# MatteoMer/zolt

Measured on AMD Instinct MI355X. Metric: BN254 G1 MSM/sec, higher is better.
Workload: dtype u32; 1 GPU; msm_g1_2^20; points=1048576, points_per_gpu=1048576, streams=3, window_bits=17, windows=15, table_levels=15, table_bytes=1006632960, mode=precomputed table of multiples

## Files before the change

### zolt_amd/csrc/g1_29.hip.h

```cpp
#pragma once
#include "fp29.hip.h"
#include "g1.hip.h"

namespace zg {

struct XYZZ29 {
    F29 x, y, zz, zzz;
};

ZG_DEV XYZZ xyzz29_to_std(const XYZZ29 &a, bool inf) {
    if (inf) return XYZZ::identity();
    XYZZ r;
    r.x = f29_to_fp(a.x); r.y = f29_to_fp(a.y); r.zz = f29_to_fp(a.zz); r.zzz = f29_to_fp(a.zzz);
    return r;
}
ZG_DEV void xyzz29_from_std(const XYZZ &s, XYZZ29 &a, bool &inf) {
    inf = s.is_identity();
    a.x = f29_from_fp(s.x); a.y = f29_from_fp(s.y); a.zz = f29_from_fp(s.zz); a.zzz = f29_from_fp(s.zzz);
}

ZG_DEV void xyzz29_start(XYZZ29 &a, const F29 &px, const F29 &py) {
    a.x = px; a.y = py;
#pragma unroll
    for (int i = 0; i < 9; i++) { a.zz.l[i] = Fp29::ONE[i]; a.zzz.l[i] = Fp29::ONE[i]; }
}

ZG_DEV u32 xyzz29_madd_nz(XYZZ29 &a, const F29 &px, const F29 &py, u32 neg) {
#ifdef ZG_F29_SERIAL
    F29 U2 = f29_mul(px, a.zz);
    F29 S2 = f29_mul(py, a.zzz);
#else
    F29 U2, S2;
    f29_mul_x2(U2, px, a.zz, S2, py, a.zzz);
#endif
    F29 Pp = f29_sub7(U2, a.x);
    F29 R = f29_pmsub45(S2, a.y, neg);
    u32 exc = 0;
#ifndef ZG_EXP_NOSLOW
    if (f29_is_zero_modp(Pp)) exc = f29_is_zero_modp(R) ? 2u : 1u;
#endif
#ifdef ZG_F29_SERIAL
    F29 PP = f29_sqr(Pp);
    F29 PPP = f29_mul(Pp, PP);
    F29 Q = f29_mul(a.x, PP);
    F29 X3 = f29_x3(f29_sqr(R), PPP, Q);
    F29 Y3 = f29_mul2(R, f29_sub7(Q, X3), f29_neg4(a.y), PPP);
    a.zz = f29_mul(a.zz, PP);
    a.zzz = f29_mul(a.zzz, PPP);
    a.x = X3;
    a.y = Y3;
#else
    F29 PP, RR, PPP, Q, ZZ3, Y3, ZZZ3;
    f29_sqr_x2(PP, Pp, RR, R);
    f29_mul_x3(PPP, Pp, PP, Q, a.x, PP, ZZ3, a.zz, PP);
    F29 X3 = f29_x3(RR, PPP, Q);
    f29_mul2_mul(Y3, R, f29_sub7(Q, X3), f29_neg4(a.y), PPP, ZZZ3, a.zzz, PPP);
    a.x = X3;
    a.y = Y3;
    a.zz = ZZ3;
    a.zzz = ZZZ3;
#endif
    return exc;
}
ZG_DEV void xyzz29_madd_except(XYZZ29 &a, bool &inf, const F29 &px, const F29 &py, u32 neg, u32 exc) {
    if (exc == 2u) {
        Affine q;
        q.x = f29_to_fp(px); q.y = f29_to_fp(neg ? f29_neg2(py) : py);
        xyzz29_from_std(xyzz_dbl_affine(q), a, inf);
    } else {
        inf = true;
    }
}

ZG_DEV void xyzz29_madd(XYZZ29 &a, bool &inf, const F29 &px, const F29 &py) {
    if (inf) {
        xyzz29_start(a, px, py);
        inf = false;
        return;
    }
    u32 exc = xyzz29_madd_nz(a, px, py, 0u);
    if (exc) xyzz29_madd_except(a, inf, px, py, 0u, exc);
}

ZG_DEV XYZZ29 xyzz29_identity() {
    XYZZ29 r;
#pragma unroll
    for (int i = 0; i < 9; i++) { r.x.l[i] = 0; r.y.l[i] = 0; r.zz.l[i] = 0; r.zzz.l[i] = 0; }
    return r;
}
ZG_DEV bool xyzz29_is_identity(const XYZZ29 &a) { return f29_all_zero(a.zz); }

ZG_DEV XYZZ29 xyzz29_from_std_val(const XYZZ &s) {
    if (s.is_identity()) return xyzz29_identity();
    XYZZ29 a;
    a.x = f29_from_fp(s.x); a.y = f29_from_fp(s.y); a.zz = f29_from_fp(s.zz); a.zzz = f29_from_fp(s.zzz);
    return a;
}
ZG_DEV XYZZ xyzz29_to_std_val(const XYZZ29 &a) { return xyzz29_to_std(a, xyzz29_is_identity(a)); }

ZG_DEV XYZZ29 xyzz29_dbl(const XYZZ29 &p) {
    if (xyzz29_is_identity(p)) return p;
    F29 U = f29_times2(p.y);
    F29 V = f29_sqr(U);
    F29 W = f29_mul(U, V);
    F29 S = f29_mul(p.x, V);
    F29 M = f29_times3(f29_sqr(p.x));
    XYZZ29 r;
    r.x = f29_sub4_2c(f29_sqr(M), S);
    r.y = f29_mul2(M, f29_sub7(S, r.x), W, f29_neg4(p.y));
    r.zz = f29_mul(V, p.zz);
    r.zzz = f29_mul(W, p.zzz);
    return r;
}

struct Jac29 {
    F29 x, y, z;
};
ZG_DEV Jac29 jac29_dbl(const Jac29 &p) {
    F29 A = f29_sqr(p.x);
    F29 B = f29_sqr(p.y);
    F29 B4 = f29_times4(B);
    F29 D = f29_mul(p.x, B4);
    F29 E = f29_times3(A);
    F29 F = f29_sqr(E);
    Jac29 r;
    r.x = f29_sub4_2c(F, D);
    r.y = f29_mul2(E, f29_sub7(D, r.x), f29_neg2(B), f29_times2(B4));
    r.z = f29_mul(f29_times2(p.y), p.z);
    return r;
}

ZG_DEV XYZZ29 xyzz29_add(const XYZZ29 &a, const XYZZ29 &b) {
    if (xyzz29_is_identity(a)) return b;
    if (xyzz29_is_identity(b)) return a;
    F29 U1 = f29_mul(a.x, b.zz);
    F29 U2 = f29_mul(b.x, a.zz);
    F29 S1 = f29_mul(a.y, b.zzz);
    F29 S2 = f29_mul(b.y, a.zzz);
    F29 Pp = f29_sub2(U2, U1);
    F29 R = f29_sub2(S2, S1);
    if (f29_is_zero_modp(Pp)) {
        if (f29_is_zero_modp(R)) return xyzz29_dbl(a);
        return xyzz29_identity();
    }
    F29 PP = f29_sqr(Pp);
    F29 PPP = f29_mul(Pp, PP);
    F29 Q = f29_mul(U1, PP);
    XYZZ29 r;
    r.x = f29_x3(f29_sqr(R), PPP, Q);
    r.y = f29_mul2(R, f29_sub7(Q, r.x), f29_neg2(S1), PPP);
    r.zz = f29_mul(f29_mul(a.zz, b.zz), PP);
    r.zzz = f29_mul(f29_mul(a.zzz, b.zzz), PPP);
    return r;
}

ZG_DEV XYZZ29 xyzz29_load(const void *p) {
    const uint4 *q = reinterpret_cast<const uint4 *>(p);
    u32 w[36];
#pragma unroll
    for (int i = 0; i < 9; i++) {
        uint4 v = q[i];
        w[4 * i] = v.x; w[4 * i + 1] = v.y; w[4 * i + 2] = v.z; w[4 * i + 3] = v.w;
    }
    XYZZ29 r;
#pragma unroll
    for (int i = 0; i < 9; i++) { r.x.l[i] = w[i]; r.y.l[i] = w[9 + i]; r.zz.l[i] = w[18 + i]; r.zzz.l[i] = w[27 + i]; }
    return r;
}
ZG_DEV void xyzz29_store(void *p, const XYZZ29 &v) {
    u32 w[36];
#pragma unroll
    for (int i = 0; i < 9; i++) { w[i] = v.x.l[i]; w[9 + i] = v.y.l[i]; w[18 + i] = v.zz.l[i]; w[27 + i] = v.zzz.l[i]; }
    uint4 *q = reinterpret_cast<uint4 *>(p);
#pragma unroll
    for (int i = 0; i < 9; i++) q[i] = make_uint4(w[4 * i], w[4 * i + 1], w[4 * i + 2], w[4 * i + 3]);
}
ZG_DEV XYZZ29 xyzz29_shfl_down(const XYZZ29 &v, int delta) {
    XYZZ29 r;
#pragma unroll
    for (int i = 0; i < 9; i++) {
        r.x.l[i] = __shfl_down(v.x.l[i], delta, 64);
        r.y.l[i] = __shfl_down(v.y.l[i], delta, 64);
        r.zz.l[i] = __shfl_down(v.zz.l[i], delta, 64);
        r.zzz.l[i] = __shfl_down(v.zzz.l[i], delta, 64);
    }
    return r;
}

}
```

### zolt_amd/csrc/msm.hip

```cpp
#include <string.h>

#include <mutex>
#include <vector>

#include "common.hip.h"
#include "g1.hip.h"
#include "g1_29.hip.h"
#include "g1_29x4.hip.h"
#include "msm_plan.h"

#ifndef ZG_TAIL_PRIO
#define ZG_TAIL_PRIO 3
#endif
#define ZG_HIPRIO() __builtin_amdgcn_s_setprio(ZG_TAIL_PRIO)

struct zg_bases_s {
    size_t n = 0;
    int device = -1;
    zg::MsmPlan plan;
    char *d_table = nullptr;
    uint8_t *d_inf = nullptr;
    uint64_t *d_scal = nullptr;
    struct Lane {
        uint32_t *d_dig = nullptr, *d_sorted = nullptr, *d_hist = nullptr, *d_starts = nullptr;
// ... 672 lines not shown
#else
#define ZG_ROW_MASK 0x7FFFFFFFu
#endif
#ifdef ZG_EXP_ACC_WAVES
#define ZG_ACC_ATTR __attribute__((amdgpu_waves_per_eu(ZG_EXP_ACC_WAVES, ZG_EXP_ACC_WAVES)))
#else
#define ZG_ACC_ATTR __attribute__((amdgpu_waves_per_eu(2, 2)))
#endif
struct Row29 {
    uint4 w[4];
};
ZG_DEV Row29 row29_load(const char *p) {
    Row29 r;
    const uint4 *q = reinterpret_cast<const uint4 *>(p);
#pragma unroll
    for (int i = 0; i < 4; i++) r.w[i] = q[i];
    return r;
}
ZG_DEV void row29_unpack(const Row29 &r, F29 &px, F29 &py) {
    const u32 x[8] = {r.w[0].x, r.w[0].y, r.w[0].z, r.w[0].w, r.w[1].x, r.w[1].y, r.w[1].z, r.w[1].w};
    const u32 y[8] = {r.w[2].x, r.w[2].y, r.w[2].z, r.w[2].w, r.w[3].x, r.w[3].y, r.w[3].z, r.w[3].w};
    px = f29_unpack(x);
    py = f29_unpack(y);
#pragma unroll
    for (int i = 0; i < 9; i++) {
        asm volatile("" : "+v"(px.l[i]));
        asm volatile("" : "+v"(py.l[i]));
    }
}

template <bool QUAD>
__global__ void __launch_bounds__(256) ZG_ACC_ATTR msm_accumulate_chunk_kernel(const uint32_t *sorted, const uint32_t *starts, const uint32_t *nzrank,
                                                                   const uint32_t *nzend, const char *table, uint32_t NK, uint32_t NT,
                                                                   char *part) {
    uint32_t i = blockIdx.x * blockDim.x + threadIdx.x, q = 0;
    if (QUAD) {
        q = i & 3;
        i >>= 2;
    }
    uint32_t total = starts[NK];
    uint32_t C = chunk_len(total, NT);
    uint64_t a64 = (uint64_t)i * C;
    if (i >= NT || a64 >= total) return;
    uint32_t a = (uint32_t)a64, b = a + C < total ? a + C : total;
    uint32_t lo = 0, hi = NK;
    while (hi - lo > 1) {
        uint32_t mid = (lo + hi) >> 1;
        if (starts[mid] <= a) lo = mid; else hi = mid;
    }
    uint32_t r = nzrank[lo], kend = starts[lo + 1];
#ifndef ZG_ACC_RUNEND_STARTS
    uint32_t knext = nzend[r + 1];
#endif
    XYZZ29 acc;
    bool acc_inf = true;
    uint32_t e = sorted[a];
    Row29 row = row29_load(table + 64 * (size_t)(e & ZG_ROW_MASK));
    uint32_t rneg = e >> 31;
    uint32_t e1 = a + 1 < b ? sorted[a + 1] : 0u;
    for (uint32_t p = a; p < b; p++) {
        F29 px, py;
#ifdef ZG_ACC_ROW_COPY
        Row29 nxt = row;
        uint32_t nneg = 0;
        if (p + 1 < b) {
            uint32_t e2 = e1;
            if (p + 2 < b) e1 = sorted[p + 2];
            nxt = row29_load(table + 64 * (size_t)(e2 & ZG_ROW_MASK));
            nneg = e2 >> 31;
        }
        row29_unpack(row, px, py);
        const uint32_t neg = 0u - rneg;
#else
        row29_unpack(row, px, py);
        const uint32_t neg = 0u - rneg;
        if (p + 1 < b) {
            uint32_t e2 = e1;
            if (p + 2 < b) e1 = sorted[p + 2];
            row = row29_load(table + 64 * (size_t)(e2 & ZG_ROW_MASK));
            rneg = e2 >> 31;
        }
#endif
        if (__builtin_expect(p == kend, 0)) {
            if (q == 0) xyzz29_store(part + 144 * (size_t)(i + r), acc_inf ? xyzz29_identity() : acc);
            acc_inf = true;
            r++;
#ifdef ZG_ACC_RUNEND_STARTS
            kend = starts[nzend[r] + 1];
#else
            asm volatile("v_mov_b32 %0, %1" : "=v"(kend) : "v"(knext));
            knext = nzend[r + 1];
#endif
        }
        uint32_t exc = 0;
        if (QUAD) {
            if (neg) py = f29_neg2(py);
            xyzz29_madd4(acc, acc_inf, px, py, q);
        } else if (__builtin_expect(acc_inf, 0)) {
            xyzz29_start(acc, px, neg ? f29_neg2(py) : py);
            acc_inf = false;
        } else {
#ifdef ZG_ACC_SIGN_BRANCH
            if (neg) py = f29_neg2(py);
            exc = xyzz29_madd_nz(acc, px, py, 0u);
        }
        if (__builtin_expect(exc != 0, 0)) xyzz29_madd_except(acc, acc_inf, px, py, 0u, exc);
#else
            exc = xyzz29_madd_nz(acc, px, py, neg);
        }
        if (__builtin_expect(exc != 0, 0)) xyzz29_madd_except(acc, acc_inf, px, py, neg, exc);
#endif
#ifdef ZG_ACC_ROW_COPY
        row = nxt;
        rneg = nneg;
#endif
    }
    if (q == 0) xyzz29_store(part + 144 * (size_t)(i + r), acc_inf ? xyzz29_identity() : acc);
}

__global__ void __launch_bounds__(64) msm_bucket_combine_kernel(const char *part, const uint32_t *starts, const uint32_t *nzrank, uint32_t NK,
                                                                uint32_t NT, int GS, char *buckets, uint32_t *heavy_list, MsmState *st) {
    ZG_HIPRIO();
    uint32_t t = (blockIdx.x * 64 + threadIdx.x) >> 2, q = threadIdx.x & 3;
    uint32_t k = t / (uint32_t)GS, g = t % (uint32_t)GS;
    XYZZ29 acc = xyzz29_identity();
    bool light = false;
    if (k < NK) {
        uint32_t C = chunk_len(starts[NK], NT);
        uint32_t s0 = starts[k], s1 = starts[k + 1];
        if (s1 == s0) {
            light = true;
        } else {
            uint32_t q0 = s0 / C, q1 = (s1 - 1) / C, cnt = q1 - q0 + 1, base = q0 + nzrank[k];
            if (cnt > 8u * (uint32_t)GS) {
                if (g == 0 && q == 0) {
                    if (cnt > HUGE_PARTIALS) heavy_list[NK + atomicAdd(&st->nhuge, 1u)] = k;
                    else heavy_list[atomicAdd(&st->nheavy, 1u)] = k;
                }
            } else {
                light = true;
                if (g < cnt) acc = xyzz29_load(part + 144 * (size_t)(base + g));
                uint32_t j = g + (uint32_t)GS;
                XYZZ29 nxt = j < cnt ? xyzz29_load(part + 144 * (size_t)(base + j)) : xyzz29_identity();
                while (j < cnt) {
                    XYZZ29 cur = nxt;
                    j += (uint32_t)GS;
                    if (j < cnt) nxt = xyzz29_load(part + 144 * (size_t)(base + j));
                    acc = xyzz29_add4(acc, cur, q);
                }
            }
        }
    }
    for (int d = 1; d < GS; d <<= 1) {
        XYZZ29 o = xyzz29_shfl_down(acc, 4 * d);
        if ((g & (uint32_t)(2 * d - 1)) == 0) acc = xyzz29_add4(acc, o, q);
    }
    if (light && g == 0 && q == 0) xyzz29_store(buckets + 144 * (size_t)k, acc);
}

__device__ __forceinline__ XYZZ29 block_sum_xyzz29(const XYZZ29 &acc, uint4 *sh) {
    uint32_t tid = threadIdx.x;
    xyzz29_store(&sh[tid * 9], acc);
    __syncthreads();
    if (tid < 128) {
        XYZZ29 x = xyzz29_load(&sh[tid * 9]), y = xyzz29_load(&sh[(tid + 128) * 9]);
        xyzz29_store(&sh[tid * 9], xyzz29_add(x, y));
    }
    __syncthreads();
    uint32_t g = tid >> 2, q = tid & 3;
    for (uint32_t o = 64; o > 0; o >>= 1) {
        if (g < o) {
            XYZZ29 x = xyzz29_load(&sh[g * 9]), y = xyzz29_load(&sh[(g + o) * 9]);
            XYZZ29 r = xyzz29_add4(x, y, q);
            if (q == 0) xyzz29_store(&sh[g * 9], r);
        }
        __syncthreads();
    }
    return xyzz29_load(&sh[0]);
}

__device__ __forceinline__ XYZZ29 wave_sum_xyzz29(const XYZZ29 &acc, uint4 *sh) {
    const uint32_t tid = threadIdx.x;
    xyzz29_store(&sh[tid * 9], acc);
    __syncthreads();
    if (tid < 32) {
        XYZZ29 x = xyzz29_load(&sh[tid * 9]), y = xyzz29_load(&sh[(tid + 32) * 9]);
        xyzz29_store(&sh[tid * 9], xyzz29_add(x, y));
    }
    __syncthreads();
    const uint32_t g = tid >> 2, q = tid & 3;
    for (uint32_t o = 16; o > 0; o >>= 1) {
        if (g < o) {
            XYZZ29 x = xyzz29_load(&sh[g * 9]), y = xyzz29_load(&sh[(g + o) * 9]);
            XYZZ29 r = xyzz29_add4(x, y, q);
            if (q == 0) xyzz29_store(&sh[g * 9], r);
        }
        __syncthreads();
    }
    return xyzz29_load(&sh[0]);
}

__global__ void __launch_bounds__(256) msm_heavy_kernel(const char *part, const uint32_t *starts, const uint32_t *nzrank, const uint32_t *nzlist,
                                                        uint32_t NK, uint32_t NT, const uint32_t *heavy_list, MsmState *st, char *part2,
                                                        char *buckets) {
    ZG_HIPRIO();
    __shared__ uint4 sh[256 * 9];
    __shared__ uint32_t sh_last;
    const uint32_t nheavy = st->nheavy, nhuge = st->nhuge;
    if (nheavy == 0 && nhuge == 0) return;
    const uint32_t C = chunk_len(starts[NK], NT), tid = threadIdx.x;
    {
        const uint32_t lane = tid & 63;
        for (uint32_t h = blockIdx.x * 4 + (tid >> 6); h < nheavy; h += gridDim.x * 4) {
            uint32_t k = heavy_list[h];
            uint32_t s0 = starts[k], s1 = starts[k + 1];
            uint32_t q0 = s0 / C, q1 = (s1 - 1) / C, cnt = q1 - q0 + 1, base = q0 + nzrank[k];
            XYZZ29 acc = xyzz29_identity();
            for (uint32_t j = lane; j < cnt; j += 64) acc = xyzz29_add(acc, xyzz29_load(part + 144 * (size_t)(base + j)));
            for (int d = 1; d < 64; d <<= 1) {
                XYZZ29 o = xyzz29_shfl_down(acc, d);
                if ((lane & (uint32_t)(2 * d - 1)) == 0) acc = xyzz29_add(acc, o);
            }
            if (lane == 0) xyzz29_store(buckets + 144 * (size_t)k, acc);
        }
    }
    if (nhuge == 0) return;
    const uint32_t *huge_list = heavy_list + NK;
    uint32_t *arrive = reinterpret_cast<uint32_t *>(st) + 4;
    uint32_t NZ = nzrank[NK];
    uint32_t lo_slot = blockIdx.x * HEAVY_BLOCK_ITEMS, hi_slot = lo_slot + HEAVY_BLOCK_ITEMS;
    if (lo_slot >= NT + NK) return;
    uint32_t lo = 0, hi = NZ;
    while (hi - lo > 1) {
        uint32_t mid = (lo + hi) >> 1;
        if (starts[nzlist[mid]] / C + mid <= lo_slot) lo = mid; else hi = mid;
    }
    for (uint32_t r = lo; r < NZ; r++) {
        uint32_t k = nzlist[r];
        uint32_t s0 = starts[k], s1 = starts[k + 1];
        uint32_t q0 = s0 / C, q1 = (s1 - 1) / C, cnt = q1 - q0 + 1, base = q0 + r;
        if (base >= hi_slot) break;
        if (cnt <= HUGE_PARTIALS || base + cnt <= lo_slot) continue;
        uint32_t r0 = base > lo_slot ? base : lo_slot, r1 = base + cnt < hi_slot ? base + cnt : hi_slot;
        XYZZ29 acc = xyzz29_identity();
        for (uint32_t j = r0 + tid; j < r1; j += 256) acc = xyzz29_add(acc, xyzz29_load(part + 144 * (size_t)j));
        XYZZ29 res = block_sum_xyzz29(acc, sh);
        const uint32_t b0 = base / HEAVY_BLOCK_ITEMS, b1 = (base + cnt - 1) / HEAVY_BLOCK_ITEMS;
        if (tid == 0) {
            xyzz29_store(part2 + 144 * (size_t)(blockIdx.x + r), res);
            uint32_t h = 0;
            while (h < nhuge && huge_list[h] != k) h++;
            uint32_t arrived = __hip_atomic_fetch_add(&arrive[h], 1u, __ATOMIC_ACQ_REL, __HIP_MEMORY_SCOPE_AGENT);
            asm volatile("s_waitcnt vmcnt(0)" ::: "memory");
            sh_last = arrived == b1 - b0 ? 1u : 0u;
        }
        __syncthreads();
        if (sh_last) {
            XYZZ29 a2 = xyzz29_identity();
            for (uint32_t bb = b0 + tid; bb <= b1; bb += 256) a2 = xyzz29_add(a2, xyzz29_load(part2 + 144 * (size_t)(bb + r)));
            __syncthreads();
            XYZZ29 tot = block_sum_xyzz29(a2, sh);
            if (tid == 0) xyzz29_store(buckets + 144 * (size_t)k, tot);
        }
        __syncthreads();
    }
}

__global__ void __launch_bounds__(256) msm_bitsum_kernel(const char *buckets, uint32_t NB, int c, char *out) {
    ZG_HIPRIO();
    __shared__ uint4 sh[256 * 9];
    uint32_t b = blockIdx.y, g = blockIdx.z, PB = gridDim.x;
    uint32_t total = (b == (uint32_t)(c - 1)) ? 1u : NB / 2;
    XYZZ29 acc = xyzz29_identity();
    for (uint32_t j = blockIdx.x * 256 + threadIdx.x; j < total; j += PB * 256) {
        uint32_t k = (b == (uint32_t)(c - 1)) ? NB : ((((j >> b) << 1) | 1u) << b) | (j & ((1u << b) - 1u));
        acc = xyzz29_add(acc, xyzz29_load(buckets + 144 * ((size_t)g * NB + (k - 1))));
    }
    XYZZ29 r = block_sum_xyzz29(acc, sh);
    if (threadIdx.x == 0) xyzz29_store(out + 144 * (((size_t)g * c + b) * PB + blockIdx.x), r);
}

__global__ void __launch_bounds__(256) msm_rowcol_kernel(const char *buckets, uint32_t NB, int lb, int hb, char *rc) {
    ZG_HIPRIO();
    __shared__ uint4 sh[256 * 9];
    const uint32_t x = blockIdx.x, g = blockIdx.y, nrow = 1u << hb, ncol = 1u << lb, t = threadIdx.x;
    XYZZ29 acc = xyzz29_identity();
    const uint32_t len = x < nrow ? ncol : nrow;
    for (uint32_t e = t; e < len; e += 256) {
        const uint32_t k = x < nrow ? ((x << lb) | e) : ((e << lb) | (x - nrow));
        if (k != 0) {
            XYZZ29 v = xyzz29_load(buckets + 144 * ((size_t)g * NB + (k - 1)));
            acc = e < 256 ? v : xyzz29_add(acc, v);
        }
    }
    XYZZ29 r = block_sum_xyzz29(acc, sh);
    if (t == 0) xyzz29_store(rc + 144 * ((size_t)g * (nrow + ncol) + x), r);
}
__global__ void __launch_bounds__(64) msm_rowcol_wave_kernel(const char *buckets, uint32_t NB, int lb, int hb, char *rc) {
    ZG_HIPRIO();
    __shared__ uint4 sh[64 * 9];
    const uint32_t x = blockIdx.x, g = blockIdx.y, nrow = 1u << hb, ncol = 1u << lb, t = threadIdx.x;
    XYZZ29 acc = xyzz29_identity();
    const uint32_t len = x < nrow ? ncol : nrow;
    bool first = true;
    for (uint32_t e = t; e < len; e += 64) {
        const uint32_t k = x < nrow ? ((x << lb) | e) : ((e << lb) | (x - nrow));
        if (k != 0) {
            XYZZ29 v = xyzz29_load(buckets + 144 * ((size_t)g * NB + (k - 1)));
            acc = first ? v : xyzz29_add(acc, v);
            first = false;
        }
    }
    XYZZ29 r = wave_sum_xyzz29(acc, sh);
    if (t == 0) xyzz29_store(rc + 144 * ((size_t)g * (nrow + ncol) + x), r);
}
static void launch_rowcol(hipStream_t st, const char *buckets, uint32_t NB, int lb, int hb, int sets, char *rc) {
    const int wave_from = env_int("ZG_MSM_ROWCOL_WAVE_FROM", 3);
    if (wave_from > 0 && sets >= wave_from)
        hipLaunchKernelGGL(msm_rowcol_wave_kernel, dim3((1u << hb) + (1u << lb), sets), dim3(64), 0, st, buckets, NB, lb, hb, rc);
    else
        hipLaunchKernelGGL(msm_rowcol_kernel, dim3((1u << hb) + (1u << lb), sets), dim3(256), 0, st, buckets, NB, lb, hb, rc);
}

__global__ void __launch_bounds__(256) msm_bits2d_kernel(const char *buckets, const char *rc, uint32_t NB, int c, int lb, int hb, char *out) {
    ZG_HIPRIO();
    __shared__ uint4 sh[256 * 9];
    const uint32_t b = blockIdx.x, g = blockIdx.y, nrow = 1u << hb, ncol = 1u << lb, t = threadIdx.x;
    const char *rcg = rc + 144 * (size_t)g * (nrow + ncol);
    XYZZ29 acc = xyzz29_identity();
    if (b == (uint32_t)(c - 1)) {
        if (t == 0) acc = xyzz29_load(buckets + 144 * ((size_t)g * NB + (NB - 1)));
    } else if (b < (uint32_t)lb) {
        for (uint32_t e = t; e < ncol; e += 256)
            if ((e >> b) & 1u) acc = xyzz29_add(acc, xyzz29_load(rcg + 144 * (size_t)(nrow + e)));
    } else {
        for (uint32_t e = t; e < nrow; e += 256)
            if ((e >> (b - (uint32_t)lb)) & 1u) acc = xyzz29_add(acc, xyzz29_load(rcg + 144 * (size_t)e));
    }
    XYZZ29 r = block_sum_xyzz29(acc, sh);
    if (t == 0) xyzz29_store(out + 144 * ((size_t)g * c + b), r);
}

ZG_DEV void write_result(const XYZZ &acc, int mode, uint64_t *out_rec, uint8_t *out_inf) {
    Affine r;
    bool inf = xyzz_to_affine(acc, r);
    if (mode == 0) {
        affine_store(out_rec, r);
        *out_inf = inf ? 1 : 0;
    } else {
        Fp one = Fp::one();
        if (inf) {
            fe_store(out_rec, one); fe_store(out_rec + 4, one); fe_store(out_rec + 8, Fp::zero());
        } else {
            fe_store(out_rec, r.x); fe_store(out_rec + 4, r.y); fe_store(out_rec + 8, one);
        }
    }
}

ZG_DEV void write_partial_unnormalised(const XYZZ &acc, uint64_t *out_rec) {
    Fp X, Y, Z;
    xyzz_to_jacobian(acc, X, Y, Z);
    fe_store(out_rec, X); fe_store(out_rec + 4, Y); fe_store(out_rec + 8, Z);
}

__global__ void __launch_bounds__(512) msm_final_kernel(const char *bits, int c, int PB, int G, char *rg, int mode, uint64_t *out_rec,
                                                        uint8_t *out_inf, uint32_t rec_stride, uint32_t inf_stride) {
    ZG_HIPRIO();
    __shared__ uint4 pts[256 * 9];
    uint32_t tid = threadIdx.x, g = blockIdx.x, quad = tid >> 2, q = tid & 3;
    uint32_t S = 1;
    while (S < (uint32_t)PB) S <<= 1;
    if (tid < 256) {
        uint32_t b = tid / S, j = tid % S;
        XYZZ29 v = xyzz29_identity();
        if (b < (uint32_t)c && j < (uint32_t)PB) v = xyzz29_load(bits + 144 * (((size_t)g * c + b) * PB + j));
        xyzz29_store(&pts[tid * 9], v);
    }
    __syncthreads();
    for (uint32_t d = 1; d < S; d <<= 1) {
        uint32_t per_bit = S / (2 * d);
        if (quad < (256 / S) * per_bit) {
            uint32_t b = quad / per_bit, j = (quad % per_bit) * 2 * d;
            XYZZ29 x = xyzz29_load(&pts[(b * S + j) * 9]), y = xyzz29_load(&pts[(b * S + j + d) * 9]);
            XYZZ29 r = xyzz29_add4(x, y, q);
            if (q == 0) xyzz29_store(&pts[(b * S + j) * 9], r);
        }
        __syncthreads();
    }
    if (quad < (uint32_t)c) {
        XYZZ29 v = xyzz29_load(&pts[(quad * S) * 9]);
#if !(defined(ZG_EXP_SKIP) && (ZG_EXP_SKIP & 1))
        for (uint32_t i = 0; i < quad; i++) v = xyzz29_dbl4(v, q);
// ... 626 lines not shown
            uint32_t *d_fbase = ln.d_fine + (size_t)items * ((size_t)1 << q.fb);
            hipLaunchKernelGGL(msm_fine_count_kernel, dim3(items), dim3(1024), 0, st, ln.d_tmp, ln.d_cstarts, d_tst, d_ist, q.NCB, q.fb, q.rb,
                               ln.d_fine);
            hipLaunchKernelGGL(msm_fine_offsets_kernel, dim3(q.NCB), dim3(128), 0, st, d_ist, q.fb, p.NK, ln.d_fine, d_fbase, ln.d_hist);
            hipLaunchKernelGGL(msm_fine_place_kernel, dim3(items), dim3(1024), (STAGE_ENTRIES + 128 + 132) * 4, st, ln.d_tmp, ln.d_cstarts, d_tst,
                               d_ist, q.NCB, q.fb, q.rb, ln.d_fine, d_fbase, sv.sorted, local_shift, (uint32_t)b->n, (uint32_t)off);
        }
        uint32_t tiles = div_up(p.NK, 1024);
        hipLaunchKernelGGL(msm_scan_a_kernel, dim3(tiles), dim3(1024), 0, st, ln.d_hist, p.NK, ln.d_scan_tmp, ln.d_scan_tmp + p.NK,
                           ln.d_scan_tmp + 2 * (size_t)p.NK);
        hipLaunchKernelGGL(msm_scan_b_kernel, dim3(tiles), dim3(1024), 0, st, ln.d_hist, p.NK, ln.d_scan_tmp, ln.d_scan_tmp + p.NK,
                           ln.d_scan_tmp + 2 * (size_t)p.NK, sv.starts, sv.nzrank, sv.nzlist, sv.nzend, reinterpret_cast<uint32_t *>(sv.state),
                           state_words(p.NT, p.NK));
    } else if (q.sort == MsmSort::LDS) {
        uint32_t per_block = (uint32_t)((n + nblk - 1) / nblk);
        prof_begin(ZG_PROF_MSM_DIGITS, st);
        ZG_TRY(launch_digits_lds_c(p.c, st, d_scalars, infp, (uint32_t)n, (uint32_t)n_pts, p.G, per_block, p.NK, nblk, ln.d_dig,
                                   ln.d_blockhist, 0, 0, rows));
        prof_end(ZG_PROF_MSM_DIGITS, st);
        prof_begin(ZG_PROF_MSM_SORT, st);
        hipLaunchKernelGGL(msm_colscan_kernel, dim3(div_up(p.NK, 256)), dim3(256), 0, st, ln.d_blockhist, nblk, p.NK, ln.d_hist);
        {
            uint32_t tiles = div_up(p.NK, 1024);
            hipLaunchKernelGGL(msm_scan_a_kernel, dim3(tiles), dim3(1024), 0, st, ln.d_hist, p.NK, ln.d_scan_tmp, ln.d_scan_tmp + p.NK,
                               ln.d_scan_tmp + 2 * (size_t)p.NK);
            hipLaunchKernelGGL(msm_scan_b_kernel, dim3(tiles), dim3(1024), 0, st, ln.d_hist, p.NK, ln.d_scan_tmp, ln.d_scan_tmp + p.NK,
                               ln.d_scan_tmp + 2 * (size_t)p.NK, sv.starts, sv.nzrank, sv.nzlist, sv.nzend, reinterpret_cast<uint32_t *>(sv.state),
                               state_words(p.NT, p.NK));
        }
        static PerDeviceOnce scatter_once;
        ZG_HIP(scatter_once.run([] {
            return hipFuncSetAttribute(reinterpret_cast<const void *>(msm_scatter_lds_kernel), hipFuncAttributeMaxDynamicSharedMemorySize, 128 * 1024);
        }));
        hipLaunchKernelGGL(msm_scatter_lds_kernel, dim3(nblk), dim3(sort_threads()), p.NK * 4, st, ln.d_dig, (uint32_t)n, (uint32_t)n_pts, p.W, p.G,
                           b->n, (uint32_t)off, per_block, p.NK, sv.starts, ln.d_blockhist, sv.sorted, rowv);
    } else {
        prof_begin(ZG_PROF_MSM_DIGITS, st);
        ZG_HIP(hipMemsetAsync(ln.d_hist, 0, (size_t)p.NK * 4, st));
        ZG_TRY(launch_digits_c(p.c, st, d_scalars, infp, (uint32_t)n, (uint32_t)n_pts, p.G, ln.d_dig, ln.d_hist));
        prof_end(ZG_PROF_MSM_DIGITS, st);
        prof_begin(ZG_PROF_MSM_SORT, st);
        {
            uint32_t tiles = div_up(p.NK, 1024);
            hipLaunchKernelGGL(msm_scan_a_kernel, dim3(tiles), dim3(1024), 0, st, ln.d_hist, p.NK, ln.d_scan_tmp, ln.d_scan_tmp + p.NK,
                               ln.d_scan_tmp + 2 * (size_t)p.NK);
            hipLaunchKernelGGL(msm_scan_b_kernel, dim3(tiles), dim3(1024), 0, st, ln.d_hist, p.NK, ln.d_scan_tmp, ln.d_scan_tmp + p.NK,
                               ln.d_scan_tmp + 2 * (size_t)p.NK, sv.starts, sv.nzrank, sv.nzlist, sv.nzend, reinterpret_cast<uint32_t *>(sv.state),
                               state_words(p.NT, p.NK));
        }
        ZG_HIP(hipMemsetAsync(ln.d_hist, 0, (size_t)p.NK * 4, st));
        hipLaunchKernelGGL(msm_scatter_kernel, dim3(div_up(n, 256), p.W), dim3(256), 0, st, ln.d_dig, (uint32_t)n, (uint32_t)n_pts, p.G,
                           b->n, (uint32_t)off, sv.starts, ln.d_hist, sv.sorted);
    }
    prof_end(ZG_PROF_MSM_SORT, st);
    return ZG_OK;
    };
    auto accumulate_range = [&](size_t n_pts, const SliceView &sv, char *bucket_out) -> int {
    const size_t n = n_pts * (size_t)p.K;
    prof_begin(ZG_PROF_MSM_ACCUMULATE, st);
    bool alone = env_int("ZG_MSM_ALONE_FULL", 1) != 0;
    for (auto &o : b->lanes)
        if (alone && &o != &ln && o.used && o.last_st != st && hipEventQuery(o.done) == hipErrorNotReady) alone = false;
    (void)hipGetLastError();
    if (p.G > 1) alone = true;
    uint32_t NT = chunk_threads((uint64_t)n * p.W, alone);
    if (NT > p.NT || forced_chunk_threads()) NT = p.NT;
    static const unsigned acc_block = [] {
        int v = env_int("ZG_MSM_ACC_BLOCK", 256);
        return (unsigned)(v == 64 || v == 128 ? v : 256);
    }();
#ifdef ZG_ACC_RUNEND_STARTS
    const uint32_t *run_ends = sv.nzlist;
#else
    const uint32_t *run_ends = sv.nzend;
#endif
    if (NT <= (uint32_t)env_int("ZG_MSM_QUAD_ACC_MAX_CHUNKS", 32768))
        hipLaunchKernelGGL(msm_accumulate_chunk_kernel<true>, dim3(div_up((size_t)NT * 4, 256)), dim3(256), 0, st, sv.sorted, sv.starts,
                           sv.nzrank, run_ends, b->d_table, p.NK, NT, ln.d_part);
    else
        hipLaunchKernelGGL(msm_accumulate_chunk_kernel<false>, dim3(div_up(NT, acc_block)), dim3(acc_block), 0, st, sv.sorted, sv.starts,
                           sv.nzrank, run_ends, b->d_table, p.NK, NT, ln.d_part);
    prof_end(ZG_PROF_MSM_ACCUMULATE, st);
    prof_begin(ZG_PROF_MSM_REDUCE, st);
    hipLaunchKernelGGL(msm_bucket_combine_kernel, dim3(div_up((size_t)p.NK * p.GS * 4, 64)), dim3(64), 0, st, ln.d_part, sv.starts,
                       sv.nzrank, p.NK, NT, p.GS, bucket_out, ln.d_heavy, reinterpret_cast<MsmState *>(sv.state));
    uint32_t nblk_a = (NT + p.NK) / HEAVY_BLOCK_ITEMS + 1;
    hipLaunchKernelGGL(msm_heavy_kernel, dim3(nblk_a < 256 ? 256 : nblk_a), dim3(256), 0, st, ln.d_part, sv.starts, sv.nzrank, sv.nzlist,
                       p.NK, NT, ln.d_heavy, reinterpret_cast<MsmState *>(sv.state), ln.d_part2, bucket_out);
    return ZG_OK;
    };
    auto view = [&](size_t j) {
        SliceView sv{ln.d_sorted, ln.d_starts, ln.d_nzrank, ln.d_nzlist, ln.d_nzend, ln.d_state};
        if (S > 1) {
            uint32_t *m = ln.d_slice_meta + j * meta_stride;
            sv = SliceView{ln.d_sorted + j * (size_t)p.W * per, m, m + ((size_t)p.NK + 1), m + 2 * ((size_t)p.NK + 1), m + 3 * ((size_t)p.NK + 1),
                           m + 4 * ((size_t)p.NK + 1)};
        }
        return sv;
    };
    for (size_t j = 0; j < S; j++) {
        const size_t a = j * per, cnt = n_pts - a < per ? n_pts - a : per;
        if (j) prof_end(ZG_PROF_MSM_REDUCE, st);
        ZG_TRY(sort_range(off + a, cnt, d_scalars + 4 * a, view(j)));
        ZG_TRY(accumulate_range(cnt, view(j), j == 0 ? (t_bucket_sink && S == 1 ? t_bucket_sink : ln.d_partial) : ln.d_slice_buckets + (j - 1) * (size_t)p.NK * 144));
    }
    if (t_bucket_sink && S == 1) {
        prof_end(ZG_PROF_MSM_REDUCE, st);
        ZG_HIP(hipGetLastError());
        ZG_HIP(hipEventRecord(ln.done, st));
        return ZG_OK;
    }
    if (S > 1)
        hipLaunchKernelGGL(msm_bucket_fold_kernel, dim3(div_up((size_t)p.NK * 4, 256)), dim3(256), 0, st, ln.d_partial, ln.d_slice_buckets, p.NK,
                           (uint32_t)S);
    if (p.lb) {
        char *d_rc = ln.d_bits + 144 * (size_t)p.G * p.K * p.c;
        launch_rowcol(st, ln.d_partial, p.NB, p.lb, p.hb, p.G * p.K, d_rc);
        hipLaunchKernelGGL(msm_bits2d_kernel, dim3(p.c, p.G * p.K), dim3(256), 0, st, ln.d_partial, d_rc, p.NB, p.c, p.lb, p.hb, ln.d_bits);
    } else {
        hipLaunchKernelGGL(msm_bitsum_kernel, dim3(p.PB, p.c, p.G * p.K), dim3(256), 0, st, ln.d_partial, p.NB, p.c, ln.d_bits);
    }
    hipLaunchKernelGGL(msm_final_kernel, dim3(p.G * p.K), dim3(512), 0, st, ln.d_bits, p.c, p.lb ? 1 : p.PB, p.G, ln.d_rg, mode, d_rec, d_inf_out,
                       rec_stride, inf_stride);
    if (p.G > 1)
        hipLaunchKernelGGL(msm_groups_kernel, dim3(p.K), dim3(4), 0, st, ln.d_rg, p.G, p.c, mode, d_rec, d_inf_out, rec_stride, inf_stride);
    prof_end(ZG_PROF_MSM_REDUCE, st);
    ZG_HIP(hipGetLastError());
    ZG_HIP(hipEventRecord(ln.done, st));
    return ZG_OK;
}

namespace hostfp {
typedef unsigned __int128 u128;
static const uint64_t P[4] = {0x3c208c16d87cfd47ull, 0x97816a916871ca8dull, 0xb85045b68181585dull, 0x30644e72e131a029ull};
static uint64_t n0inv() {
    uint64_t inv = 1;
    for (int i = 0; i < 6; i++) inv *= 2 - P[0] * inv;
    return 0 - inv;
}
static void mul(uint64_t r[4], const uint64_t a[4], const uint64_t b[4]) {
    static const uint64_t N0 = n0inv();
    uint64_t t[6] = {0, 0, 0, 0, 0, 0};
    for (int i = 0; i < 4; i++) {
        u128 c = 0;
        for (int j = 0; j < 4; j++) {
            c += (u128)a[j] * b[i] + t[j];
            t[j] = (uint64_t)c;
            c >>= 64;
        }
        c += t[4];
        t[4] = (uint64_t)c;
        t[5] = (uint64_t)(c >> 64);
        const uint64_t m = t[0] * N0;
        c = ((u128)m * P[0] + t[0]) >> 64;
        for (int j = 1; j < 4; j++) {
            c += (u128)m * P[j] + t[j];
            t[j - 1] = (uint64_t)c;
            c >>= 64;
        }
        c += t[4];
        t[3] = (uint64_t)c;
        t[4] = t[5] + (uint64_t)(c >> 64);
    }
    uint64_t d[4];
    u128 br = 0;
    for (int j = 0; j < 4; j++) {
        u128 v = (u128)t[j] - P[j] - (uint64_t)br;
        d[j] = (uint64_t)v;
// ... 692 lines not shown
```

### zolt_amd/csrc/msm_plan.h

```cpp
#pragma once
#include <stdint.h>
#include <stdlib.h>

#include <string>

#include "../../include/zolt_gpu.h"

namespace zg {

void set_error(const std::string &msg);

static constexpr int MAX_GROUPS = 64;
static constexpr uint64_t MAX_BUCKETS = (uint64_t)1 << 21;
static constexpr size_t LDS_SORT_BYTES = 128 * 1024;
static constexpr int ENTRY_BITS = 31;
static constexpr int FINE_BITS_MAX = 7;
static constexpr int FINE_BITS_MIN = 5;
static constexpr uint32_t COARSE_BINS_MAX = 3000;
static constexpr uint32_t TWO_PASS_MIN_BUCKETS = 8192;
static constexpr uint32_t FINE_SLICE = 32768;
static constexpr size_t DEV_SLICES_MAX = 128;
static_assert((uint64_t)COARSE_BINS_MAX << FINE_BITS_MAX <= MAX_BUCKETS && LDS_SORT_BYTES / 4 <= MAX_BUCKETS, "fused sets stay plannable");

enum class MsmSort { ATOMIC, LDS, TWO_PASS };

struct MsmPlan {
    int c;
    int W;
    int L;
    int G;
    uint32_t NB;
    uint32_t NK;
    int K;
    int PB;
    int lb, hb;
    uint32_t NT;
    int GS;
    MsmSort sort;
    int fb;
    int rb;
    uint32_t NCB;
    uint32_t nblk;
};

static inline size_t ceil_div(size_t a, size_t b) { return (a + b - 1) / b; }

static inline int env_int(const char *name, int dflt) {
    const char *v = getenv(name);
    return v && *v ? atoi(v) : dflt;
}

static inline uint32_t forced_chunk_threads() {
    int v = env_int("ZG_MSM_CHUNK_THREADS", 0);
    return v < 1 ? 0u : (uint32_t)v;
}

static inline uint32_t sort_span(uint32_t NK) {
    int v = env_int("ZG_MSM_SORT_SPAN", 0);
    if (v > 0) return (uint32_t)v;
    return NK <= 4096 ? 256u : 2048u;
}

static inline uint32_t two_pass_span(int W) {
    uint32_t cap = W <= 16 ? 2048u : 1024u;
    uint32_t v = (uint32_t)env_int("ZG_MSM_TWO_PASS_SPAN", 2048);
    v = v < 256 ? 256 : v;
    return v > cap ? cap : v;
}

static inline uint32_t chunk_threads(uint64_t digits, bool alone = false) {
    static const uint64_t per_chunk = [] {
        int v = env_int("ZG_MSM_CHUNK_ENTRIES", 16);
        return (uint64_t)(v < 1 ? 1 : v);
    }();
    uint64_t want = digits / per_chunk;
    uint32_t nt = 1024;
    while (nt < want && nt < 131072u) nt <<= 1;
    static const uint32_t inflight = [] {
        int v = env_int("ZG_MSM_INFLIGHT_CHUNKS", 114688);
        return (uint32_t)(v < 1024 ? 1024 : (v > 131072 ? 131072 : v));
    }();
    return nt == 131072u && !alone ? inflight : nt;
}

static int plan_shape(size_t n, const zg_msm_config *cfg, size_t batch, MsmPlan &p) {
    int c = cfg ? cfg->window_bits : 0;
    if (c == 0) c = env_int("ZG_MSM_WINDOW_BITS", 0);
    int L = cfg ? cfg->precompute_levels : 0;
    if (L == 0) L = env_int("ZG_MSM_PRECOMPUTE", 0);
    if (L == 0 && cfg && cfg->expected_uses > 0 && cfg->expected_uses < 16) L = 1;
    if (c == 0 && L == 1) {
        c = n >= ((size_t)1 << 19) ? 15 : (n >= 8192 ? 13 : (n >= 2048 ? 8 : (n >= 64 ? 7 : 5)));
    }
    if (c == 0) {
        c = n >= 32768 ? 16 : (n >= 8192 ? 10 : (n >= 2048 ? 8 : (n >= 64 ? 7 : 5)));
        if (batch == 1 && n >= (size_t)env_int("ZG_MSM_C17_MIN", 900000) && (uint64_t)n * 15 <= ((uint64_t)1 << (ENTRY_BITS - FINE_BITS_MIN))) c = 17;
    }
    if (c < 2 || c > 19) {
        set_error("msm: window_bits must be in [2,19]");
        return ZG_ERR_INVALID;
    }
    p.c = c;
    p.W = (255 + c - 1) / c;
    if (L == 0) L = p.W;
    if (L < 1) L = 1;
    if (L > p.W) L = p.W;
    p.G = (p.W + L - 1) / L;
    p.L = (p.W + p.G - 1) / p.G;
    if (p.G > MAX_GROUPS) {
        set_error("msm: too many bucket groups for this window size");
        return ZG_ERR_INVALID;
    }
    p.NB = 1u << (c - 1);
    p.K = (int)batch;
    if ((uint64_t)p.NB * p.G * batch > MAX_BUCKETS) {
        set_error("msm: too many buckets");
        return ZG_ERR_INVALID;
    }
    p.NK = p.NB * (uint32_t)p.G * (uint32_t)batch;
    const uint32_t forced = forced_chunk_threads();
    p.NT = forced ? forced : chunk_threads((uint64_t)n * batch * p.W, true);
    p.GS = 1;
    const uint64_t nt_usual = forced ? p.NT : chunk_threads((uint64_t)n * batch * p.W);
    while (p.GS < 16 && (uint64_t)p.GS * (uint64_t)env_int("ZG_MSM_COMBINE_PER_QUAD", 4) < nt_usual / p.NK + 1) p.GS <<= 1;
    int pb = (int)(p.NB / 2 / (256 * 4));
    p.PB = pb < 1 ? 1 : (pb > 16 ? 16 : pb);
    if (c > 16 && p.PB > 8) p.PB = 8;
    p.lb = p.hb = 0;
    if (c >= 11 && env_int("ZG_MSM_REDUCE_2D", 1)) {
        p.lb = c / 2;
        p.hb = c - 1 - p.lb;
    }
    return ZG_OK;
}

static inline int fine_bits(size_t table_rows, int fb_max) {
    int need = 1;
    while (((size_t)1 << need) < table_rows) need++;
    return ENTRY_BITS - need < fb_max ? ENTRY_BITS - need : fb_max;
}

static void plan_sort(MsmPlan &p, size_t table_rows, size_t n_total, bool fused) {
    p.fb = p.rb = 0;
    p.NCB = 0;
    if (env_int("ZG_MSM_TWO_PASS_SORT", 1) && p.NK >= TWO_PASS_MIN_BUCKETS && p.W <= 32 && (uint64_t)n_total * p.W >= (1u << 17)) {
        int fb_max = env_int("ZG_MSM_FINE_BITS", FINE_BITS_MAX);
        const int fb = fine_bits(table_rows, fb_max > FINE_BITS_MAX ? FINE_BITS_MAX : fb_max);
        const uint32_t ncb = fb >= env_int("ZG_MSM_FINE_BITS_MIN", FINE_BITS_MIN) ? (p.NK + (1u << fb) - 1) >> fb : 0;
        if (ncb && ncb <= COARSE_BINS_MAX) {
            p.sort = MsmSort::TWO_PASS;
            p.fb = fb;
            p.rb = ENTRY_BITS - fb;
            p.NCB = ncb;
            const uint32_t nblk = (uint32_t)ceil_div(n_total, two_pass_span(p.W));
            p.nblk = nblk < 1 ? 1 : nblk;
            return;
        }
    }
    if ((size_t)p.NK * 4 <= LDS_SORT_BYTES && (fused || env_int("ZG_MSM_LDS_SORT", 1))) {
        p.sort = MsmSort::LDS;
        const uint32_t nblk = (uint32_t)(n_total / (size_t)sort_span(p.NK));
        p.nblk = nblk < 1 ? 1 : (nblk > 256 ? 256 : nblk);
        return;
    }
    p.sort = MsmSort::ATOMIC;
    p.nblk = 0;
}

static int plan_msm(size_t n, const zg_msm_config *cfg, size_t k, size_t table_n, MsmPlan &p, const MsmPlan *within = nullptr) {
    const int rc = plan_shape(n ? n : 1, cfg, k, p);
    if (rc != ZG_OK) return rc;
    if (!within) {
        plan_sort(p, (size_t)p.L * table_n, n * k, k > 1);
        return ZG_OK;
    }
    p.sort = within->sort;
    p.fb = within->fb;
    p.rb = within->rb;
    p.NCB = p.fb ? (p.NK + (1u << p.fb) - 1) >> p.fb : 0;
    p.nblk = within->nblk;
    return ZG_OK;
}

static inline size_t table_span_points(int L) {
    const size_t span_mb = (size_t)env_int("ZG_MSM_TABLE_SPAN_MB", 1024);
    if (!span_mb) return 0;
    const size_t pts = (span_mb << 20) / (64 * (size_t)L), least = (size_t)env_int("ZG_MSM_TABLE_SPAN_MIN_POINTS", 65536);
    return pts < least ? least : pts;
}
static inline void slice_counts(const MsmPlan &p, size_t n_pts, size_t &S, size_t &per) {
    S = 1;
    per = n_pts;
    if (p.K != 1) return;
    const size_t sp = table_span_points(p.L);
    if (!sp || n_pts < 2 * sp) return;
    S = (n_pts + sp - 1) / sp;
    if (S > DEV_SLICES_MAX) S = DEV_SLICES_MAX;
    per = (n_pts + S - 1) / S;
    S = (n_pts + per - 1) / per;
}
static bool slice_sort_plan(const MsmPlan &p, size_t per, MsmPlan &ps, int &shift) {
    shift = 0;
    ps = p;
    if (!env_int("ZG_MSM_SLICE_LOCAL_REFS", 1)) return false;
    int k = 1;
    while (((size_t)1 << k) < per) k++;
    plan_sort(ps, (size_t)p.L << k, per, false);
// ... 58 lines not shown
```

Before: 861.1 MSM/s.

## Batch field multiplies in reduction adds and drop identity selects in accumulate

Adds xyzz29_add_lane, which interleaves independent field multiplications via the x2/x3 multi-mul helpers, and uses it in the heavy, block-sum and bucket-reduce kernels. The accumulate path now starts a bucket with a branchless signed zzz in place of negating y, and skips the identity select on store by explicitly zeroing the accumulator in the exception path. An optional per-lane bucket combine kernel is added behind an environment variable that is off by default. The goal is more instruction-level parallelism and fewer selects, in exchange for higher register pressure in the reduction kernels.

```diff
diff --git a/zolt_amd/csrc/g1_29.hip.h b/zolt_amd/csrc/g1_29.hip.h
--- a/zolt_amd/csrc/g1_29.hip.h
+++ b/zolt_amd/csrc/g1_29.hip.h
@@ -23,6 +23,26 @@
     a.x = px; a.y = py;
 #pragma unroll
     for (int i = 0; i < 9; i++) { a.zz.l[i] = Fp29::ONE[i]; a.zzz.l[i] = Fp29::ONE[i]; }
+}
+
+constexpr F29 f29_minus_one() {
+    F29 r{};
+    u32 borrow = 0;
+    for (int i = 0; i < 9; i++) {
+        const u32 d = Fp29::P[i] - Fp29::ONE[i] - borrow;
+        borrow = d >> 31;
+        r.l[i] = i < 8 ? d & Fp29::MASK : d;
+    }
+    return r;
+}
+ZG_DEV void xyzz29_start_signed(XYZZ29 &a, const F29 &px, const F29 &py, u32 neg) {
+    constexpr F29 M = f29_minus_one();
+    a.x = px; a.y = py;
+#pragma unroll
+    for (int i = 0; i < 9; i++) {
+        a.zz.l[i] = Fp29::ONE[i];
+        a.zzz.l[i] = Fp29::ONE[i] ^ (neg & (Fp29::ONE[i] ^ M.l[i]));
+    }
 }
 
 ZG_DEV u32 xyzz29_madd_nz(XYZZ29 &a, const F29 &px, const F29 &py, u32 neg) {
@@ -69,6 +89,13 @@
         xyzz29_from_std(xyzz_dbl_affine(q), a, inf);
     } else {
         inf = true;
+#pragma unroll
+        for (int i = 0; i < 9; i++) {
+            asm volatile("v_mov_b32 %0, 0" : "=v"(a.x.l[i]));
+            asm volatile("v_mov_b32 %0, 0" : "=v"(a.y.l[i]));
+            asm volatile("v_mov_b32 %0, 0" : "=v"(a.zz.l[i]));
+            asm volatile("v_mov_b32 %0, 0" : "=v"(a.zzz.l[i]));
+        }
     }
 }
 
@@ -154,6 +181,27 @@
     return r;
 }
 
+ZG_DEV XYZZ29 xyzz29_add_lane(const XYZZ29 &a, const XYZZ29 &b) {
+    if (xyzz29_is_identity(a)) return b;
+    if (xyzz29_is_identity(b)) return a;
+    F29 U1, U2, S1, S2, ZZm, ZZZm;
+    f29_mul_x3(U1, a.x, b.zz, U2, b.x, a.zz, S1, a.y, b.zzz);
+    f29_mul_x3(S2, b.y, a.zzz, ZZm, a.zz, b.zz, ZZZm, a.zzz, b.zzz);
+    F29 Pp = f29_sub2(U2, U1);
+    F29 R = f29_sub2(S2, S1);
+    if (f29_is_zero_modp(Pp)) {
+        if (f29_is_zero_modp(R)) return xyzz29_dbl(a);
+        return xyzz29_identity();
+    }
+    F29 PP, RR, PPP, Q;
+    XYZZ29 r;
+    f29_sqr_x2(PP, Pp, RR, R);
+    f29_mul_x3(PPP, Pp, PP, Q, U1, PP, r.zz, ZZm, PP);
+    r.x = f29_x3(RR, PPP, Q);
+    f29_mul2_mul(r.y, R, f29_sub7(Q, r.x), f29_neg2(S1), PPP, r.zzz, ZZZm, PPP);
+    return r;
+}
+
 ZG_DEV XYZZ29 xyzz29_load(const void *p) {
     const uint4 *q = reinterpret_cast<const uint4 *>(p);
     u32 w[36];
diff --git a/zolt_amd/csrc/msm.hip b/zolt_amd/csrc/msm.hip
--- a/zolt_amd/csrc/msm.hip
+++ b/zolt_amd/csrc/msm.hip
@@ -778,7 +778,7 @@
         }
 #endif
         if (__builtin_expect(p == kend, 0)) {
-            if (q == 0) xyzz29_store(part + 144 * (size_t)(i + r), acc_inf ? xyzz29_identity() : acc);
+            if (q == 0) xyzz29_store(part + 144 * (size_t)(i + r), QUAD && acc_inf ? xyzz29_identity() : acc);
             acc_inf = true;
             r++;
 #ifdef ZG_ACC_RUNEND_STARTS
@@ -793,7 +793,7 @@
             if (neg) py = f29_neg2(py);
             xyzz29_madd4(acc, acc_inf, px, py, q);
         } else if (__builtin_expect(acc_inf, 0)) {
-            xyzz29_start(acc, px, neg ? f29_neg2(py) : py);
+            xyzz29_start_signed(acc, px, py, neg);
             acc_inf = false;
         } else {
 #ifdef ZG_ACC_SIGN_BRANCH
@@ -811,7 +811,7 @@
         rneg = nneg;
 #endif
     }
-    if (q == 0) xyzz29_store(part + 144 * (size_t)(i + r), acc_inf ? xyzz29_identity() : acc);
+    if (q == 0) xyzz29_store(part + 144 * (size_t)(i + r), QUAD && acc_inf ? xyzz29_identity() : acc);
 }
 
 __global__ void __launch_bounds__(64) msm_bucket_combine_kernel(const char *part, const uint32_t *starts, const uint32_t *nzrank, uint32_t NK,
@@ -854,13 +854,41 @@
     if (light && g == 0 && q == 0) xyzz29_store(buckets + 144 * (size_t)k, acc);
 }
 
+__global__ void __launch_bounds__(64) msm_bucket_combine_lane_kernel(const char *part, const uint32_t *starts, const uint32_t *nzrank, uint32_t NK,
+                                                                     uint32_t NT, int GS, char *buckets, uint32_t *heavy_list, MsmState *st) {
+    ZG_HIPRIO();
+    const uint32_t k = blockIdx.x * 64 + threadIdx.x;
+    if (k >= NK) return;
+    const uint32_t C = chunk_len(starts[NK], NT);
+    const uint32_t s0 = starts[k], s1 = starts[k + 1];
+    XYZZ29 acc = xyzz29_identity();
+    if (s1 != s0) {
+        const uint32_t q0 = s0 / C, q1 = (s1 - 1) / C, cnt = q1 - q0 + 1, base = q0 + nzrank[k];
+        if (cnt > 8u * (uint32_t)GS) {
+            if (cnt > HUGE_PARTIALS) heavy_list[NK + atomicAdd(&st->nhuge, 1u)] = k;
+            else heavy_list[atomicAdd(&st->nheavy, 1u)] = k;
+            return;
+        }
+        acc = xyzz29_load(part + 144 * (size_t)base);
+        uint32_t j = 1;
+        XYZZ29 nxt = j < cnt ? xyzz29_load(part + 144 * (size_t)(base + j)) : xyzz29_identity();
+        while (j < cnt) {
+            XYZZ29 cur = nxt;
+            j++;
+            if (j < cnt) nxt = xyzz29_load(part + 144 * (size_t)(base + j));
+            acc = xyzz29_add_lane(acc, cur);
+        }
+    }
+    xyzz29_store(buckets + 144 * (size_t)k, acc);
+}
+
 __device__ __forceinline__ XYZZ29 block_sum_xyzz29(const XYZZ29 &acc, uint4 *sh) {
     uint32_t tid = threadIdx.x;
     xyzz29_store(&sh[tid * 9], acc);
     __syncthreads();
     if (tid < 128) {
         XYZZ29 x = xyzz29_load(&sh[tid * 9]), y = xyzz29_load(&sh[(tid + 128) * 9]);
-        xyzz29_store(&sh[tid * 9], xyzz29_add(x, y));
+        xyzz29_store(&sh[tid * 9], xyzz29_add_lane(x, y));
     }
     __syncthreads();
     uint32_t g = tid >> 2, q = tid & 3;
@@ -881,7 +909,7 @@
     __syncthreads();
     if (tid < 32) {
         XYZZ29 x = xyzz29_load(&sh[tid * 9]), y = xyzz29_load(&sh[(tid + 32) * 9]);
-        xyzz29_store(&sh[tid * 9], xyzz29_add(x, y));
+        xyzz29_store(&sh[tid * 9], xyzz29_add_lane(x, y));
     }
     __syncthreads();
     const uint32_t g = tid >> 2, q = tid & 3;
@@ -912,7 +940,7 @@
             uint32_t s0 = starts[k], s1 = starts[k + 1];
             uint32_t q0 = s0 / C, q1 = (s1 - 1) / C, cnt = q1 - q0 + 1, base = q0 + nzrank[k];
             XYZZ29 acc = xyzz29_identity();
-            for (uint32_t j = lane; j < cnt; j += 64) acc = xyzz29_add(acc, xyzz29_load(part + 144 * (size_t)(base + j)));
+            for (uint32_t j = lane; j < cnt; j += 64) acc = xyzz29_add_lane(acc, xyzz29_load(part + 144 * (size_t)(base + j)));
             for (int d = 1; d < 64; d <<= 1) {
                 XYZZ29 o = xyzz29_shfl_down(acc, d);
                 if ((lane & (uint32_t)(2 * d - 1)) == 0) acc = xyzz29_add(acc, o);
@@ -939,7 +967,7 @@
         if (cnt <= HUGE_PARTIALS || base + cnt <= lo_slot) continue;
         uint32_t r0 = base > lo_slot ? base : lo_slot, r1 = base + cnt < hi_slot ? base + cnt : hi_slot;
         XYZZ29 acc = xyzz29_identity();
-        for (uint32_t j = r0 + tid; j < r1; j += 256) acc = xyzz29_add(acc, xyzz29_load(part + 144 * (size_t)j));
+        for (uint32_t j = r0 + tid; j < r1; j += 256) acc = xyzz29_add_lane(acc, xyzz29_load(part + 144 * (size_t)j));
         XYZZ29 res = block_sum_xyzz29(acc, sh);
         const uint32_t b0 = base / HEAVY_BLOCK_ITEMS, b1 = (base + cnt - 1) / HEAVY_BLOCK_ITEMS;
         if (tid == 0) {
@@ -953,7 +981,7 @@
         __syncthreads();
         if (sh_last) {
             XYZZ29 a2 = xyzz29_identity();
-            for (uint32_t bb = b0 + tid; bb <= b1; bb += 256) a2 = xyzz29_add(a2, xyzz29_load(part2 + 144 * (size_t)(bb + r)));
+            for (uint32_t bb = b0 + tid; bb <= b1; bb += 256) a2 = xyzz29_add_lane(a2, xyzz29_load(part2 + 144 * (size_t)(bb + r)));
             __syncthreads();
             XYZZ29 tot = block_sum_xyzz29(a2, sh);
             if (tid == 0) xyzz29_store(buckets + 144 * (size_t)k, tot);
@@ -970,7 +998,7 @@
     XYZZ29 acc = xyzz29_identity();
     for (uint32_t j = blockIdx.x * 256 + threadIdx.x; j < total; j += PB * 256) {
         uint32_t k = (b == (uint32_t)(c - 1)) ? NB : ((((j >> b) << 1) | 1u) << b) | (j & ((1u << b) - 1u));
-        acc = xyzz29_add(acc, xyzz29_load(buckets + 144 * ((size_t)g * NB + (k - 1))));
+        acc = xyzz29_add_lane(acc, xyzz29_load(buckets + 144 * ((size_t)g * NB + (k - 1))));
     }
     XYZZ29 r = block_sum_xyzz29(acc, sh);
     if (threadIdx.x == 0) xyzz29_store(out + 144 * (((size_t)g * c + b) * PB + blockIdx.x), r);
@@ -986,7 +1014,7 @@
         const uint32_t k = x < nrow ? ((x << lb) | e) : ((e << lb) | (x - nrow));
         if (k != 0) {
             XYZZ29 v = xyzz29_load(buckets + 144 * ((size_t)g * NB + (k - 1)));
-            acc = e < 256 ? v : xyzz29_add(acc, v);
+            acc = e < 256 ? v : xyzz29_add_lane(acc, v);
         }
     }
     XYZZ29 r = block_sum_xyzz29(acc, sh);
@@ -1003,7 +1031,7 @@
         const uint32_t k = x < nrow ? ((x << lb) | e) : ((e << lb) | (x - nrow));
         if (k != 0) {
             XYZZ29 v = xyzz29_load(buckets + 144 * ((size_t)g * NB + (k - 1)));
-            acc = first ? v : xyzz29_add(acc, v);
+            acc = first ? v : xyzz29_add_lane(acc, v);
             first = false;
         }
     }
@@ -1796,8 +1824,12 @@
                            sv.nzrank, run_ends, b->d_table, p.NK, NT, ln.d_part);
     prof_end(ZG_PROF_MSM_ACCUMULATE, st);
     prof_begin(ZG_PROF_MSM_REDUCE, st);
-    hipLaunchKernelGGL(msm_bucket_combine_kernel, dim3(div_up((size_t)p.NK * p.GS * 4, 64)), dim3(64), 0, st, ln.d_part, sv.starts,
-                       sv.nzrank, p.NK, NT, p.GS, bucket_out, ln.d_heavy, reinterpret_cast<MsmState *>(sv.state));
+    if (p.combine_lane)
+        hipLaunchKernelGGL(msm_bucket_combine_lane_kernel, dim3(div_up((size_t)p.NK, 64)), dim3(64), 0, st, ln.d_part, sv.starts, sv.nzrank,
+                           p.NK, NT, p.GS, bucket_out, ln.d_heavy, reinterpret_cast<MsmState *>(sv.state));
+    else
+        hipLaunchKernelGGL(msm_bucket_combine_kernel, dim3(div_up((size_t)p.NK * p.GS * 4, 64)), dim3(64), 0, st, ln.d_part, sv.starts,
+                           sv.nzrank, p.NK, NT, p.GS, bucket_out, ln.d_heavy, reinterpret_cast<MsmState *>(sv.state));
     uint32_t nblk_a = (NT + p.NK) / HEAVY_BLOCK_ITEMS + 1;
     hipLaunchKernelGGL(msm_heavy_kernel, dim3(nblk_a < 256 ? 256 : nblk_a), dim3(256), 0, st, ln.d_part, sv.starts, sv.nzrank, sv.nzlist,
                        p.NK, NT, ln.d_heavy, reinterpret_cast<MsmState *>(sv.state), ln.d_part2, bucket_out);
diff --git a/zolt_amd/csrc/msm_plan.h b/zolt_amd/csrc/msm_plan.h
--- a/zolt_amd/csrc/msm_plan.h
+++ b/zolt_amd/csrc/msm_plan.h
@@ -36,6 +36,7 @@
     int lb, hb;
     uint32_t NT;
     int GS;
+    bool combine_lane;
     MsmSort sort;
     int fb;
     int rb;
@@ -83,6 +84,8 @@
     return nt == 131072u && !alone ? inflight : nt;
 }
 
+static inline bool combine_by_lane() { return env_int("ZG_MSM_COMBINE_LANE", 0) != 0; }
+
 static int plan_shape(size_t n, const zg_msm_config *cfg, size_t batch, MsmPlan &p) {
     int c = cfg ? cfg->window_bits : 0;
     if (c == 0) c = env_int("ZG_MSM_WINDOW_BITS", 0);
@@ -123,6 +126,7 @@
     p.GS = 1;
     const uint64_t nt_usual = forced ? p.NT : chunk_threads((uint64_t)n * batch * p.W);
     while (p.GS < 16 && (uint64_t)p.GS * (uint64_t)env_int("ZG_MSM_COMBINE_PER_QUAD", 4) < nt_usual / p.NK + 1) p.GS <<= 1;
+    p.combine_lane = combine_by_lane();
     int pb = (int)(p.NB / 2 / (256 * 4));
     p.PB = pb < 1 ? 1 : (pb > 16 ? 16 : pb);
     if (c > 16 && p.PB > 8) p.PB = 8;
```

Result: no change. 862.6 MSM/s (median of 6 runs) (+0.2%).
